# yandex/pire

Measured on NVIDIA H100. Metric: scanned GB/s, higher is better.
Workload: dtype u8

## Files before the change

pire_b200/csrc/scan_kernels.cu:

```cuda

#include "scan_kernels.cuh"

#include <atomic>
#include <mutex>
#include <cstdlib>
#include <type_traits>

#include <cooperative_groups.h>
#include <cub/device/device_radix_sort.cuh>
#include <cub/device/device_scan.cuh>
#include <cub/device/device_select.cuh>
#include <cub/iterator/counting_input_iterator.cuh>

extern "C" {
extern __shared__ __align__(1024) uint8_t pire_b200_smem[];
}

namespace pire_b200 {

namespace {

constexpr int kBlock = 512;
constexpr int kMinBlocksPerSM = 3;
constexpr int kGenericBlocksPerSM = 2;
// ... 527 lines not shown

    for (uint32_t unit = blockIdx.x * warps_per_block + (threadIdx.x >> 5); unit < units; unit += warps) {
        uint32_t g, prev;
        bool known;
        {
            const uint64_t i = (uint64_t) unit * 32 + (threadIdx.x & 31);
            const uint8_t* p = a.corpus + (i < a.n ? i : a.n - 1) * (uint64_t) len;
            const uint32_t start = LaneStart<kStarts>(a, t, i, i < a.n, known);
            prev = start;
            g = start < t.H ? start : t.H;
            if (blocks != 0) {
                uint4 a0, a1, b0, b1;
                LoadStream32(p, a0, a1);
                for (uint32_t left = blocks;;) {
                    const bool more_b = left > 1;
                    p += 32;
                    if (more_b)
                        LoadStream32(p, b0, b1);
                    __syncwarp();
                    LookBlock32<k64, kClean>(t, g, prev, a0, a1, b0.x, more_b, f, a.opaque_zero, &a);
                    if (!more_b)
                        break;
                    const bool more_a = left > 2;
                    p += 32;
                    if (more_a)
                        LoadStream32(p, a0, a1);
                    __syncwarp();
                    LookBlock32<k64, kClean>(t, g, prev, b0, b1, a0.x, more_a, f, a.opaque_zero, &a);
                    left -= 2;
                    if (!more_a || __all_sync(0xffffffffu, sv.noexit[g] != 0))
                        break;
                }
            }
        }
        const uint64_t i = (uint64_t) unit * 32 + (threadIdx.x & 31);
        LaneState s;
        s.g = t.H;
        s.cold = g == t.H ? prev : g;
        Report(a, t, s, unit, i, i < a.n, known);
    }
}

template <bool kClean>
__device__ __forceinline__ void LookWord2(uint32_t& ga, uint32_t wa, uint32_t bba0, uint32_t paa0, uint32_t pana, uint32_t basea,
                                          const LookFilter& fa, uint32_t& gb, uint32_t wb, uint32_t bbb0, uint32_t pab0, uint32_t panb,
                                          uint32_t baseb, const LookFilter& fb)
{
    uint32_t bba1, bba2, bba3, paa1, paa2, paa3, bbb1, bbb2, bbb3, pab1, pab2, pab3;
    LookProbe<false, 1, kClean>(wa, basea, fa, bba1, paa1);
    LookProbe<false, 1, kClean>(wb, baseb, fb, bbb1, pab1);
    LookStep<kClean>(ga, bba0, paa0, paa1);
    LookStep<kClean>(gb, bbb0, pab0, pab1);
    LookProbe<false, 2, kClean>(wa, basea, fa, bba2, paa2);
    LookProbe<false, 2, kClean>(wb, baseb, fb, bbb2, pab2);
    LookStep<kClean>(ga, bba1, paa1, paa2);
    LookStep<kClean>(gb, bbb1, pab1, pab2);
    LookProbe<false, 3, kClean>(wa, basea, fa, bba3, paa3);
    LookProbe<false, 3, kClean>(wb, baseb, fb, bbb3, pab3);
    LookStep<kClean>(ga, bba2, paa2, paa3);
    LookStep<kClean>(gb, bbb2, pab2, pab3);
    LookStep<kClean>(ga, bba3, paa3, pana);
    LookStep<kClean>(gb, bbb3, pab3, panb);
}

template <bool kClean, uint32_t kAtB, typename Late>
__device__ __forceinline__ void LookBlock32x2(const Tables& ta, const LookFilter& fa, const ScanArgs* argsa, uint32_t& ga, uint32_t& preva,
                                              const uint4& a0, const uint4& a1, const Tables& tb, const LookFilter& fb,
                                              const ScanArgs* argsb, uint32_t& gb, uint32_t& prevb, const uint4& b0, const uint4& b1,
                                              bool more, Late late)
{
    preva = ga == ta.H ? preva : ga;
    prevb = gb == tb.H ? prevb : gb;
    uint32_t bba, paa, bna, pna, bbb, pab, bnb, pnb;
    LookProbe<false, 0, kClean>(a0.x, ta.base, fa, bba, paa);
    LookProbe<false, 0, kClean>(b0.x, tb.base, fb, bbb, pab);
    LookProbe<false, 0, kClean>(a0.y, ta.base, fa, bna, pna);
    LookProbe<false, 0, kClean>(b0.y, tb.base, fb, bnb, pnb);
    LookWord2<kClean>(ga, a0.x, bba, paa, pna, ta.base, fa, gb, b0.x, bbb, pab, pnb, tb.base, fb);
    LookProbe<false, 0, kClean>(a0.z, ta.base, fa, bba, paa);
    LookProbe<false, 0, kClean>(b0.z, tb.base, fb, bbb, pab);
    LookWord2<kClean>(ga, a0.y, bna, pna, paa, ta.base, fa, gb, b0.y, bnb, pnb, pab, tb.base, fb);
    LookProbe<false, 0, kClean>(a0.w, ta.base, fa, bna, pna);
    LookProbe<false, 0, kClean>(b0.w, tb.base, fb, bnb, pnb);
    LookWord2<kClean>(ga, a0.z, bba, paa, pna, ta.base, fa, gb, b0.z, bbb, pab, pnb, tb.base, fb);
    LookProbe<false, 0, kClean>(a1.x, ta.base, fa, bba, paa);
    LookProbe<false, 0, kClean>(b1.x, tb.base, fb, bbb, pab);
    LookWord2<kClean>(ga, a0.w, bna, pna, paa, ta.base, fa, gb, b0.w, bnb, pnb, pab, tb.base, fb);
    LookProbe<false, 0, kClean>(a1.y, ta.base, fa, bna, pna);
    LookProbe<false, 0, kClean>(b1.y, tb.base, fb, bnb, pnb);
    LookWord2<kClean>(ga, a1.x, bba, paa, pna, ta.base, fa, gb, b1.x, bbb, pab, pnb, tb.base, fb);
    LookProbe<false, 0, kClean>(a1.z, ta.base, fa, bba, paa);
    LookProbe<false, 0, kClean>(b1.z, tb.base, fb, bbb, pab);
    LookWord2<kClean>(ga, a1.y, bna, pna, paa, ta.base, fa, gb, b1.y, bnb, pnb, pab, tb.base, fb);
    LookProbe<false, 0, kClean>(a1.w, ta.base, fa, bna, pna);
    LookProbe<false, 0, kClean>(b1.w, tb.base, fb, bnb, pnb);
    LookWord2<kClean>(ga, a1.z, bba, paa, pna, ta.base, fa, gb, b1.z, bbb, pab, pnb, tb.base, fb);
    uint32_t latea, lateb;
    late(ga, gb, latea, lateb);
    LookProbe<false, 0, kClean>(latea, ta.base, fa, bba, paa);
    LookProbe<false, 0, kClean>(lateb, tb.base, fb, bbb, pab);
    LookWord2<kClean>(ga, a1.w, bna, pna, more ? paa : 0x80000000u, ta.base, fa, gb, b1.w, bnb, pnb, more ? pab : 0x80000000u, tb.base,
                      fb);
    if (ga == ta.H) {
        preva = ReplayBlock32(argsa, preva, a0, a1);
        ga = preva < ta.H ? preva : ta.H;
    }
    if (gb == tb.H) {
        prevb = ReplayBlock32<kAtB>(argsb, prevb, b0, b1);
        gb = prevb < tb.H ? prevb : tb.H;
    }
}

template <bool kClean, typename Late>
__device__ __forceinline__ void LookBlock32x2(const Tables& t, uint32_t& ga, uint32_t& preva, const uint4& a0, const uint4& a1,
                                              uint32_t& gb, uint32_t& prevb, const uint4& b0, const uint4& b1, bool more,
                                              const LookFilter& f, Late late, const ScanArgs* args)
{
    LookBlock32x2<kClean, 0>(t, f, args, ga, preva, a0, a1, t, f, args, gb, prevb, b0, b1, more, late);
}

constexpr int kRingBlock = 768;
constexpr uint32_t kRingSlots = 3;
constexpr uint32_t kRingSlotBytes = 2048;
constexpr size_t kRingWarpBytes = (size_t) kRingSlots * kRingSlotBytes;

__device__ __forceinline__ uint32_t NextSlot(uint32_t slot) { return slot + kRingSlotBytes == kRingWarpBytes ? 0 : slot + kRingSlotBytes; }

__device__ __forceinline__ void CopyBlock32(uint32_t dst_shared, const uint8_t* src)
{
    asm volatile("cp.async.cg.shared.global.L2::128B [%0], [%1], 16;\n\t"
                 "cp.async.cg.shared.global [%2], [%3], 16;" ::"r"(dst_shared), "l"(src), "r"(dst_shared + 512), "l"(src + 16)
                 : "memory");
}

__device__ __forceinline__ uint32_t LoadShared4(uint32_t shared_addr)
{
    uint32_t v;
    asm volatile("ld.shared.u32 %0, [%1];" : "=r"(v) : "r"(shared_addr) : "memory");
    return v;
}

struct RingNext {
    uint32_t at;
    uint32_t zero;
    __device__ __forceinline__ void operator()(uint32_t ga, uint32_t gb, uint32_t& latea, uint32_t& lateb) const
    {
        CopyAsyncWait<kRingSlots - 1>();
        latea = LoadShared4(at + ga * zero);
        lateb = LoadShared4(at + 1024 + gb * zero);
    }
};

template <bool kStarts>
__device__ __forceinline__ void LookRingScan(const ScanArgs& a)
{
    uint8_t* const smem = pire_b200_smem;
    SharedView sv = CarveShared(smem, a.hot);
    StageTables(a, sv, a.hot8, a.hot);

    Tables t;
    t.hot = sv.hot;
    t.base = SmemWindowBase();
    t.cls = sv.cls;
    t.full = a.full;
    t.H = a.hot;
    t.letters = a.letters;
    t.wide = a.wide;
    t.m0 = a.look_bitmap;
    LookFilter f;
    f.lo = a.look_bitmap;
    f.hi = 0;
    f.zero = a.opaque_zero;
    f.rev = __brev(f.lo);

    const uint32_t units = (uint32_t) ((a.n + 31) / 32);
    const uint32_t pairs = (units + 1) / 2;
    const uint32_t warps_per_block = blockDim.x >> 5;
    const uint32_t warps = gridDim.x * warps_per_block;
    const uint32_t len = (uint32_t) a.fixed_len;
    const uint32_t blocks = len >> 5;
    const uint32_t ring = SmemAddr(sv.stage) + (threadIdx.x >> 5) * (uint32_t) kRingWarpBytes + (threadIdx.x & 31) * 16;

    for (uint32_t pair = blockIdx.x * warps_per_block + (threadIdx.x >> 5); pair < pairs; pair += warps) {
        const bool second = 2 * pair + 1 < units;
        uint32_t ga, preva, gb, prevb;
        bool knowna, knownb;
        {
            const uint64_t ia = (uint64_t) pair * 64 + (threadIdx.x & 31);
            const uint64_t ib = ia + (second ? 32 : 0);
            const uint8_t* pa = a.corpus + (ia < a.n ? ia : a.n - 1) * (uint64_t) len;
            const uint8_t* pb = a.corpus + (ib < a.n ? ib : a.n - 1) * (uint64_t) len;
            if constexpr (kStarts) {
                preva = LaneStart<true>(a, t, ia, ia < a.n, knowna);
                prevb = LaneStart<true>(a, t, ib, ib < a.n, knownb);
                ga = preva < t.H ? preva : t.H;
                gb = prevb < t.H ? prevb : t.H;
            } else {
                knowna = knownb = true;
                preva = prevb = a.start;
                ga = gb = a.start < t.H ? a.start : t.H;
            }
            if (blocks != 0) {
#pragma unroll
                for (uint32_t j = 0; j < kRingSlots; ++j) {
                    if (j < blocks) {
                        CopyBlock32(ring + j * kRingSlotBytes, pa + 32 * j);
                        CopyBlock32(ring + j * kRingSlotBytes + 1024, pb + 32 * j);
                    }
                    CopyAsyncCommit();
                }
                CopyAsyncWait<kRingSlots - 1>();
                uint32_t s0 = 0;
                for (uint32_t k = 0;; k += 2) {
                    const uint32_t s1 = NextSlot(s0);
                    uint4 a0 = LoadShared16(ring + s0), a1 = LoadShared16(ring + s0 + 512);
                    uint4 b0 = LoadShared16(ring + s0 + 1024), b1 = LoadShared16(ring + s0 + 1536);
                    if (k + kRingSlots < blocks) {
                        CopyBlock32(ring + s0, pa + 32 * (size_t) (k + kRingSlots));
                        CopyBlock32(ring + s0 + 1024, pb + 32 * (size_t) (k + kRingSlots));
                    }
                    CopyAsyncCommit();
                    const bool more_1 = k + 1 < blocks;
                    LookBlock32x2<true>(t, ga, preva, a0, a1, gb, prevb, b0, b1, more_1, f, RingNext{ring + s1, a.opaque_zero}, &a);
                    if (!more_1)
                        break;
                    const uint32_t s2 = NextSlot(s1);
                    a0 = LoadShared16(ring + s1), a1 = LoadShared16(ring + s1 + 512);
                    b0 = LoadShared16(ring + s1 + 1024), b1 = LoadShared16(ring + s1 + 1536);
                    if (k + 1 + kRingSlots < blocks) {
                        CopyBlock32(ring + s1, pa + 32 * (size_t) (k + 1 + kRingSlots));
                        CopyBlock32(ring + s1 + 1024, pb + 32 * (size_t) (k + 1 + kRingSlots));
                    }
                    CopyAsyncCommit();
                    const bool more_2 = k + 2 < blocks;
                    LookBlock32x2<true>(t, ga, preva, a0, a1, gb, prevb, b0, b1, more_2, f, RingNext{ring + s2, a.opaque_zero}, &a);
                    if (!more_2 || __all_sync(0xffffffffu, (sv.noexit[ga] & sv.noexit[gb]) != 0))
                        break;
                    s0 = s2;
                }
                CopyAsyncWait<0>();
            }
        }
        const uint64_t ia = (uint64_t) pair * 64 + (threadIdx.x & 31);
        LaneState s;
        s.g = t.H;
        s.cold = ga == t.H ? preva : ga;
        Report(a, t, s, 2 * (uint64_t) pair, ia, ia < a.n, knowna);
        if (second) {
            s.cold = gb == t.H ? prevb : gb;
            Report(a, t, s, 2 * (uint64_t) pair + 1, ia + 32, ia + 32 < a.n, knownb);
        }
    }
}

__global__ void __launch_bounds__(kRingBlock, 1) ScanUniformLookRingKernel(const __grid_constant__ ScanArgs a) { LookRingScan<false>(a); }

__global__ void __launch_bounds__(kRingBlock, 1) ScanUniformLookRingFromKernel(const __grid_constant__ ScanArgs a) { LookRingScan<true>(a); }

constexpr int kRing1Block = 1024;
constexpr int kRing1Slots = 3;
constexpr uint32_t kRing1SlotBytes = 1024;
template <int kSlots>
__device__ __forceinline__ uint32_t NextSlot1(uint32_t slot) { return slot + kRing1SlotBytes == kSlots * kRing1SlotBytes ? 0 : slot + kRing1SlotBytes; }

template <int kSlots>
struct RingNext1 {
    uint32_t at;
    uint32_t zero;
    __device__ __forceinline__ uint32_t operator()(uint32_t g) const
    {
        CopyAsyncWait<kSlots - 1>();
        return LoadShared4(at + g * zero);
    }
};

template <int kSlots, bool kStarts>
__global__ void __launch_bounds__(kRing1Block, 1) ScanUniformLookRing1Kernel(const __grid_constant__ ScanArgs a)
{
    uint8_t* const smem = pire_b200_smem;
    SharedView sv = CarveShared(smem, a.hot);
    StageTables(a, sv, a.hot8, a.hot);

    Tables t;
    t.hot = sv.hot;
    t.base = SmemWindowBase();
    t.cls = sv.cls;
    t.full = a.full;
    t.H = a.hot;
    t.letters = a.letters;
    t.wide = a.wide;
    t.m0 = a.look_bitmap;
    LookFilter f;
    f.lo = a.look_bitmap;
    f.hi = 0;
    f.zero = a.opaque_zero;
    f.rev = __brev(f.lo);

    const uint32_t units = (uint32_t) ((a.n + 31) / 32);
    const uint32_t warps_per_block = blockDim.x >> 5;
    const uint32_t warps = gridDim.x * warps_per_block;
    const uint32_t len = (uint32_t) a.fixed_len;
    const uint32_t blocks = len >> 5;
    const uint32_t ring = SmemAddr(sv.stage) + (threadIdx.x >> 5) * (uint32_t) (kSlots * kRing1SlotBytes) + (threadIdx.x & 31) * 16;

    for (uint32_t unit = blockIdx.x * warps_per_block + (threadIdx.x >> 5); unit < units; unit += warps) {
        uint32_t g, prev;
        bool known;
        {
            const uint64_t i = (uint64_t) unit * 32 + (threadIdx.x & 31);
            const uint8_t* p = a.corpus + (i < a.n ? i : a.n - 1) * (uint64_t) len;
            const uint32_t start = LaneStart<kStarts>(a, t, i, i < a.n, known);
            prev = start;
            g = start < t.H ? start : t.H;
            if (blocks != 0) {
#pragma unroll
                for (uint32_t j = 0; j < kSlots; ++j) {
                    if (j < blocks)
                        CopyBlock32(ring + j * kRing1SlotBytes, p + 32 * j);
                    CopyAsyncCommit();
                }
                CopyAsyncWait<kSlots - 1>();
                uint32_t s0 = 0;
                for (uint32_t k = 0;; k += 2) {
                    const uint32_t s1 = NextSlot1<kSlots>(s0);
                    uint4 v0 = LoadShared16(ring + s0), v1 = LoadShared16(ring + s0 + 512);
                    if (k + kSlots < blocks)
                        CopyBlock32(ring + s0, p + 32 * (size_t) (k + kSlots));
                    CopyAsyncCommit();
                    const bool more_1 = k + 1 < blocks;
                    LookBlock32<false, true>(t, g, prev, v0, v1, more_1, f, RingNext1<kSlots>{ring + s1, a.opaque_zero}, &a);
                    if (!more_1)
                        break;
                    const uint32_t s2 = NextSlot1<kSlots>(s1);
                    v0 = LoadShared16(ring + s1), v1 = LoadShared16(ring + s1 + 512);
                    if (k + 1 + kSlots < blocks)
                        CopyBlock32(ring + s1, p + 32 * (size_t) (k + 1 + kSlots));
                    CopyAsyncCommit();
                    const bool more_2 = k + 2 < blocks;
                    LookBlock32<false, true>(t, g, prev, v0, v1, more_2, f, RingNext1<kSlots>{ring + s2, a.opaque_zero}, &a);
                    if (!more_2 || __all_sync(0xffffffffu, sv.noexit[g] != 0))
                        break;
                    s0 = s2;
                }
                CopyAsyncWait<0>();
            }
        }
        const uint64_t i = (uint64_t) unit * 32 + (threadIdx.x & 31);
        LaneState s;
        s.g = t.H;
        s.cold = g == t.H ? prev : g;
        Report(a, t, s, unit, i, i < a.n, known);
    }
}

struct PairArgs {
    ScanArgs s[2];
};
constexpr int kPairBlock = 768;
constexpr int kPairSlots = 3;
constexpr uint32_t kPairSecond = ((kMaxHot + 1 + 3) / 4 * 4 * kHotStride + 512 + 256 + 16 + 255) / 256 * 256;

struct RingPairNext {
    uint32_t at;
    uint32_t zero;
    __device__ __forceinline__ void operator()(uint32_t ga, uint32_t gb, uint32_t& latea, uint32_t& lateb) const
    {
        CopyAsyncWait<kPairSlots - 1>();
        latea = LoadShared4(at + ga * zero);
        lateb = latea + gb * zero;
    }
};

__device__ __forceinline__ void PairTables(const ScanArgs& a, const SharedView& sv, uint32_t base, Tables& t, LookFilter& f)
{
    t.hot = sv.hot;
    t.base = base;
    t.cls = sv.cls;
    t.full = a.full;
    t.H = a.hot;
    t.letters = a.letters;
    t.wide = a.wide;
    t.m0 = a.look_bitmap;
    f.lo = a.look_bitmap;
    f.hi = 0;
    f.zero = a.opaque_zero;
    f.rev = __brev(f.lo);
}

__global__ void __launch_bounds__(kPairBlock, 1) ScanPairKernel(const __grid_constant__ PairArgs p)
{
    const ScanArgs& a = p.s[0];
    const ScanArgs& b = p.s[1];
    uint8_t* const smem = pire_b200_smem;
    const SharedView sva = CarveShared(smem, a.hot);
    const SharedView svb = CarveShared(smem + kPairSecond, b.hot);
    StageTables(a, sva, a.hot8, a.hot);
    StageTables(b, svb, b.hot8, b.hot);

    Tables ta, tb;
    LookFilter fa, fb;
    PairTables(a, sva, SmemWindowBase(), ta, fa);
    PairTables(b, svb, SmemWindowBase() + kPairSecond, tb, fb);

    const uint32_t units = (uint32_t) ((a.n + 31) / 32);
    const uint32_t warps_per_block = blockDim.x >> 5;
    const uint32_t warps = gridDim.x * warps_per_block;
    const uint32_t len = (uint32_t) a.fixed_len;
    const uint32_t blocks = len >> 5;
    const uint32_t ring = SmemAddr(svb.stage) + (threadIdx.x >> 5) * (uint32_t) (kPairSlots * kRing1SlotBytes) + (threadIdx.x & 31) * 16;

    for (uint32_t unit = blockIdx.x * warps_per_block + (threadIdx.x >> 5); unit < units; unit += warps) {
        uint32_t ga, preva, gb, prevb;
        bool knowna, knownb;
        {
            const uint64_t i = (uint64_t) unit * 32 + (threadIdx.x & 31);
            const uint8_t* q = a.corpus + (i < a.n ? i : a.n - 1) * (uint64_t) len;
            preva = LaneStart<true>(a, ta, i, i < a.n && a.starts, knowna);
            prevb = LaneStart<true>(b, tb, i, i < b.n && b.starts, knownb);
            ga = preva < ta.H ? preva : ta.H;
            gb = prevb < tb.H ? prevb : tb.H;
            if (blocks != 0) {
#pragma unroll
                for (uint32_t j = 0; j < kPairSlots; ++j) {
                    if (j < blocks)
                        CopyBlock32(ring + j * kRing1SlotBytes, q + 32 * j);
                    CopyAsyncCommit();
                }
                CopyAsyncWait<kPairSlots - 1>();
                uint32_t s0 = 0;
                for (uint32_t k = 0;; k += 2) {
                    const uint32_t s1 = NextSlot1<kPairSlots>(s0);
                    uint4 v0 = LoadShared16(ring + s0), v1 = LoadShared16(ring + s0 + 512);
                    if (k + kPairSlots < blocks)
                        CopyBlock32(ring + s0, q + 32 * (size_t) (k + kPairSlots));
                    CopyAsyncCommit();
                    const bool more_1 = k + 1 < blocks;
                    LookBlock32x2<true, kPairSecond>(ta, fa, &a, ga, preva, v0, v1, tb, fb, &b, gb, prevb, v0, v1, more_1,
                                                     RingPairNext{ring + s1, a.opaque_zero});
                    if (!more_1)
                        break;
                    const uint32_t s2 = NextSlot1<kPairSlots>(s1);
                    v0 = LoadShared16(ring + s1), v1 = LoadShared16(ring + s1 + 512);
                    if (k + 1 + kPairSlots < blocks)
                        CopyBlock32(ring + s1, q + 32 * (size_t) (k + 1 + kPairSlots));
                    CopyAsyncCommit();
                    const bool more_2 = k + 2 < blocks;
                    LookBlock32x2<true, kPairSecond>(ta, fa, &a, ga, preva, v0, v1, tb, fb, &b, gb, prevb, v0, v1, more_2,
                                                     RingPairNext{ring + s2, a.opaque_zero});
                    if (!more_2 || __all_sync(0xffffffffu, (sva.noexit[ga] & svb.noexit[gb]) != 0))
                        break;
                    s0 = s2;
                }
                CopyAsyncWait<0>();
            }
        }
        const uint64_t i = (uint64_t) unit * 32 + (threadIdx.x & 31);
        LaneState s;
        s.g = ta.H;
        s.cold = ga == ta.H ? preva : ga;
        Report(a, ta, s, unit, i, i < a.n, knowna);
        s.g = tb.H;
        s.cold = gb == tb.H ? prevb : gb;
        Report(b, tb, s, unit, i, i < b.n, knownb);
    }
}

__device__ __forceinline__ uint4 LoadEdge16(const uint8_t* aligned)
{
    uint4 v;
    asm volatile("ld.global.nc.v4.u32 {%0,%1,%2,%3}, [%4];" : "=r"(v.x), "=r"(v.y), "=r"(v.z), "=r"(v.w) : "l"(aligned));
    return v;
}

struct EdgeBytes {
    uint64_t lo, hi;
    __device__ __forceinline__ EdgeBytes(uint4 v, uint32_t skip)
    {
        lo = (uint64_t) v.x | ((uint64_t) v.y << 32);
        hi = (uint64_t) v.z | ((uint64_t) v.w << 32);
        if (skip >= 8) {
            lo = hi;
            hi = 0;
            skip -= 8;
        }
        if (skip) {
            lo = (lo >> (8 * skip)) | (hi << (64 - 8 * skip));
            hi >>= 8 * skip;
        }
    }
    __device__ __forceinline__ uint32_t Next()
    {
        uint32_t b = (uint32_t) lo & 0xffu;
        lo = (lo >> 8) | (hi << 56);
        hi >>= 8;
        return b;
    }
    __device__ __forceinline__ uint4 Words() const
    {
        return make_uint4((uint32_t) lo, (uint32_t) (lo >> 32), (uint32_t) hi, (uint32_t) (hi >> 32));
    }
};

template <bool kPred>
__device__ __forceinline__ void EdgeFast(const Tables& t, LaneState& s, uint4 v, uint32_t n)
{
    const uint32_t before = s.g;
    uint32_t g = before;
    const uint32_t words = n >> 2, rest = n & 3;
    if (words > 0)
        FastWord<kPred>(t, g, v.x);
    if (words > 1)
        FastWord<kPred>(t, g, v.y);
    if (words > 2)
        FastWord<kPred>(t, g, v.z);
    if (words > 3)
        FastWord<kPred>(t, g, v.w);
    const uint32_t last = words == 0 ? v.x : words == 1 ? v.y : words == 2 ? v.z : v.w;
    if (rest > 0)
        FastStep<kPred>(t, g, last, 0x5540);
    if (rest > 1)
        FastStep<kPred>(t, g, last, 0x5541);
    if (rest > 2)
        FastStep<kPred>(t, g, last, 0x5542);
    s.g = g;
    if (g == t.H) {
        uint32_t full = before == t.H ? s.cold : before;
        EdgeBytes eb(v, 0);
        for (uint32_t k = 0; k < n; ++k)
            full = SlowStep(t, full, eb.Next());
        SetFull(t, s, full);
    }
}

__device__ __noinline__ uint4 LoadEdge16Clipped(const uint8_t* aligned, uintptr_t buf_lo, uintptr_t buf_hi)
{
    uint32_t w[4] = {0, 0, 0, 0};
    for (int k = 0; k < 16; ++k) {
        const uintptr_t at = reinterpret_cast<uintptr_t>(aligned) + k;
        if (at >= buf_lo && at < buf_hi)
            w[k >> 2] |= (uint32_t) aligned[k] << (8 * (k & 3));
    }
    return make_uint4(w[0], w[1], w[2], w[3]);
}

__device__ __forceinline__ uint4 LoadChunk16(const uint8_t* aligned, uintptr_t buf_lo, uintptr_t buf_hi)
{
    if (reinterpret_cast<uintptr_t>(aligned) >= buf_lo && reinterpret_cast<uintptr_t>(aligned) + 16 <= buf_hi)
        return LoadEdge16(aligned);
    return LoadEdge16Clipped(aligned, buf_lo, buf_hi);
}

__device__ __forceinline__ void Chunk16Look(const Tables& t, LaneState& s, uint4 v, const LookFilter& f)
{
    const uint32_t before = s.g;
    uint32_t g = s.g;
    uint32_t bb, pa, bn, pn;
    LookProbe<false, 0>(v.x, t.base, f, bb, pa);
    LookProbe<false, 0>(v.y, t.base, f, bn, pn);
    LookWord<false>(g, v.x, bb, pa, pn, t.base, f);
    LookProbe<false, 0>(v.z, t.base, f, bb, pa);
    LookWord<false>(g, v.y, bn, pn, pa, t.base, f);
    LookProbe<false, 0>(v.w, t.base, f, bn, pn);
    LookWord<false>(g, v.z, bb, pa, pn, t.base, f);
    LookWord<false>(g, v.w, bn, pn, 0xffffffffu, t.base, f);
    s.g = g;
    if (g == t.H) {
        uint32_t from = before == t.H ? s.cold : before;
        uint32_t full = ReplayChunk(t.hot, t.cls, t.full, t.H, t.letters | (t.wide << 31), from, v);
        SetFull(t, s, full);
    }
}

template <int kMode, bool kStarts>
__global__ void __launch_bounds__(kBlock, kGenericBlocksPerSM) ScanGenericKernel(const __grid_constant__ ScanArgs a)
{
    constexpr bool kPred = kMode != 0;
    LookFilter look;
    look.lo = a.look_bitmap;
    look.hi = 0;
    look.zero = 0;
    look.rev = 0;
    uint8_t* const smem = pire_b200_smem;
    SharedView sv = CarveShared(smem, a.hot);
    StageTables(a, sv, a.hot8, a.hot);

    Tables t;
    t.hot = sv.hot;
    t.base = SmemAddr(sv.hot);
    t.cls = sv.cls;
    t.full = a.full;
    t.H = a.hot;
    t.letters = a.letters;
    t.wide = a.wide;
    t.m0 = a.exit_bitmap0;

    const uint32_t lane = threadIdx.x & 31;
    const uint64_t units = (a.n + 31) / 32;
    const uint64_t warps = (uint64_t) gridDim.x * kWarpsPerBlock;
    const uint32_t stage = SmemAddr(sv.stage) + (((threadIdx.x >> 5) * kStageSlots) * 32 + lane) * 16;
    const uintptr_t buf_lo = reinterpret_cast<uintptr_t>(a.corpus);
    const uintptr_t buf_hi = buf_lo + (a.offsets ? a.offsets[a.n] - a.trim : a.n * a.fixed_len);
    const uint64_t split_first = a.split_count ? *a.split_count : 0;

    for (uint64_t unit = (uint64_t) blockIdx.x * kWarpsPerBlock + (threadIdx.x >> 5);; unit += warps) {
        if (a.work_counter) {
            unsigned int claimed = 0;
            if (lane == 0)
                claimed = atomicAdd(a.work_counter, 1u);
            unit = __shfl_sync(0xffffffffu, claimed, 0);
        }
        if (unit >= units)
            break;
        const uint64_t slot = unit * 32 + lane;
        const bool valid = slot < a.n && slot >= split_first;
        const uint64_t i = valid && a.order ? a.order[slot] : slot;
        uint64_t b = 0, e = 0;
        if (valid) {
            if (a.offsets) {
                b = a.offsets[i];
                e = a.offsets[i + 1] - a.trim;
                e = e < b ? b : e;
            } else {
                b = i * a.fixed_len;
                e = b + a.fixed_len;
            }
        }
        const uint8_t* p = a.corpus + b;
        const uint8_t* end = a.corpus + e;

        LaneState s;
        bool known;
        SetFull(t, s, LaneStart<kStarts>(a, t, i, valid, known));

        {
            const uint32_t misalign = (uint32_t) (reinterpret_cast<uintptr_t>(p) & 15);
            if (p < end && misalign != 0) {
                const uint64_t room = (uint64_t) (end - p);
                const uint32_t nhead = room < 16 - misalign ? (uint32_t) room : 16 - misalign;
                const uint8_t* chunk = p - misalign;
                if (reinterpret_cast<uintptr_t>(chunk) >= buf_lo && reinterpret_cast<uintptr_t>(chunk) + 16 <= buf_hi) {
                    EdgeFast<kPred>(t, s, EdgeBytes(LoadEdge16(chunk), misalign).Words(), nhead);
                } else {
                    uint32_t full = FullState(t, s);
                    for (uint32_t k = 0; k < nhead; ++k)
                        full = SlowStep(t, full, p[k]);
                    SetFull(t, s, full);
                }
                p += nhead;
            }
        }
        const uint32_t chunks = (uint32_t) ((end - p) >> 4);
        bool parked = false;
#pragma unroll
        for (int j = 0; j < kStageSlots; ++j) {
// ... 3542 lines not shown
```

Before: 2331.

## Stream cp.async ring continuously across units and prefetch next lane start

The per-warp copy ring now keeps feeding blocks from the next unit's strings instead of draining and re-priming at each unit boundary, so the async copies overlap the tail of one unit with the head of the next. The LaneStart lookup for the next unit is issued early, and unit assignment changes to interleave warps across blocks. Early-exit paths must wait for outstanding copies and re-prime, which adds bookkeeping and register pressure.

```diff
diff --git a/pire_b200/csrc/scan_kernels.cu b/pire_b200/csrc/scan_kernels.cu
--- a/pire_b200/csrc/scan_kernels.cu
+++ b/pire_b200/csrc/scan_kernels.cu
@@ -853,54 +853,81 @@
     const uint32_t len = (uint32_t) a.fixed_len;
     const uint32_t blocks = len >> 5;
     const uint32_t ring = SmemAddr(sv.stage) + (threadIdx.x >> 5) * (uint32_t) (kSlots * kRing1SlotBytes) + (threadIdx.x & 31) * 16;
-
-    for (uint32_t unit = blockIdx.x * warps_per_block + (threadIdx.x >> 5); unit < units; unit += warps) {
-        uint32_t g, prev;
-        bool known;
-        {
-            const uint64_t i = (uint64_t) unit * 32 + (threadIdx.x & 31);
-            const uint8_t* p = a.corpus + (i < a.n ? i : a.n - 1) * (uint64_t) len;
-            const uint32_t start = LaneStart<kStarts>(a, t, i, i < a.n, known);
-            prev = start;
-            g = start < t.H ? start : t.H;
-            if (blocks != 0) {
+    const uint32_t first = (threadIdx.x >> 5) * gridDim.x + blockIdx.x;
+    auto string_at = [&](uint32_t unit) {
+        const uint64_t i = (uint64_t) unit * 32 + (threadIdx.x & 31);
+        return a.corpus + (i < a.n ? i : a.n - 1) * (uint64_t) len;
+    };
+
+    uint32_t cunit = first, left = blocks;
+    const uint8_t* src = string_at(first);
+    auto feed = [&](uint32_t slot) {
+        if (cunit < units) {
+            CopyBlock32(slot, src);
+            src += 32;
+            if (--left == 0) {
+                cunit += warps;
+                left = blocks;
+                src = string_at(cunit);
+            }
+        }
+        CopyAsyncCommit();
+    };
+    auto prime = [&]() {
 #pragma unroll
-                for (uint32_t j = 0; j < kSlots; ++j) {
-                    if (j < blocks)
-                        CopyBlock32(ring + j * kRing1SlotBytes, p + 32 * j);
-                    CopyAsyncCommit();
+        for (uint32_t j = 0; j < kSlots; ++j)
+            feed(ring + j * kRing1SlotBytes);
+    };
+    uint32_t s0 = 0;
+    if (blocks != 0)
+        prime();
+
+    bool known;
+    uint32_t start = LaneStart<kStarts>(a, t, (uint64_t) first * 32 + (threadIdx.x & 31), (uint64_t) first * 32 + (threadIdx.x & 31) < a.n, known);
+    for (uint32_t unit = first; unit < units; unit += warps) {
+        const uint64_t i = (uint64_t) unit * 32 + (threadIdx.x & 31);
+        bool known_next;
+        const uint64_t i_next = i + 32 * (uint64_t) warps;
+        const uint32_t start_next = LaneStart<kStarts>(a, t, i_next, i_next < a.n, known_next);
+        uint32_t prev = start;
+        uint32_t g = start < t.H ? start : t.H;
+        if (blocks != 0) {
+            CopyAsyncWait<kSlots - 1>();
+            for (uint32_t k = 0;; k += 2) {
+                const uint32_t s1 = NextSlot1<kSlots>(s0);
+                uint4 v0 = LoadShared16(ring + s0), v1 = LoadShared16(ring + s0 + 512);
+                feed(ring + s0);
+                const bool more_1 = k + 1 < blocks;
+                LookBlock32<false, true>(t, g, prev, v0, v1, more_1, f, RingNext1<kSlots>{ring + s1, a.opaque_zero}, &a);
+                if (!more_1) {
+                    s0 = s1;
+                    break;
                 }
-                CopyAsyncWait<kSlots - 1>();
-                uint32_t s0 = 0;
-                for (uint32_t k = 0;; k += 2) {
-                    const uint32_t s1 = NextSlot1<kSlots>(s0);
-                    uint4 v0 = LoadShared16(ring + s0), v1 = LoadShared16(ring + s0 + 512);
-                    if (k + kSlots < blocks)
-                        CopyBlock32(ring + s0, p + 32 * (size_t) (k + kSlots));
-                    CopyAsyncCommit();
-                    const bool more_1 = k + 1 < blocks;
-                    LookBlock32<false, true>(t, g, prev, v0, v1, more_1, f, RingNext1<kSlots>{ring + s1, a.opaque_zero}, &a);
-                    if (!more_1)
-                        break;
-                    const uint32_t s2 = NextSlot1<kSlots>(s1);
-                    v0 = LoadShared16(ring + s1), v1 = LoadShared16(ring + s1 + 512);
-                    if (k + 1 + kSlots < blocks)
-                        CopyBlock32(ring + s1, p + 32 * (size_t) (k + 1 + kSlots));
-                    CopyAsyncCommit();
-                    const bool more_2 = k + 2 < blocks;
-                    LookBlock32<false, true>(t, g, prev, v0, v1, more_2, f, RingNext1<kSlots>{ring + s2, a.opaque_zero}, &a);
-                    if (!more_2 || __all_sync(0xffffffffu, sv.noexit[g] != 0))
-                        break;
-                    s0 = s2;
+                const uint32_t s2 = NextSlot1<kSlots>(s1);
+                v0 = LoadShared16(ring + s1), v1 = LoadShared16(ring + s1 + 512);
+                feed(ring + s1);
+                const bool more_2 = k + 2 < blocks;
+                LookBlock32<false, true>(t, g, prev, v0, v1, more_2, f, RingNext1<kSlots>{ring + s2, a.opaque_zero}, &a);
+                s0 = s2;
+                if (!more_2)
+                    break;
+                if (__all_sync(0xffffffffu, sv.noexit[g] != 0)) {
+                    CopyAsyncWait<0>();
+                    cunit = unit + warps;
+                    left = blocks;
+                    src = string_at(cunit);
+                    prime();
+                    s0 = 0;
+                    break;
                 }
-                CopyAsyncWait<0>();
-            }
-        }
-        const uint64_t i = (uint64_t) unit * 32 + (threadIdx.x & 31);
+            }
+        }
         LaneState s;
         s.g = t.H;
         s.cold = g == t.H ? prev : g;
         Report(a, t, s, unit, i, i < a.n, known);
+        start = start_next;
+        known = known_next;
     }
 }
 
```

Result: faster. 2360, median of 6 (+1.2%).
